# ezrakhuzadi/FFmpeg-hybrid

Hardware: AMD Instinct MI355X
Metric: decoded frames/sec (bit-exact) 4K VP9 Profile-0 @ 1/2/4/8 MI355X; % HBM roofline (higher is better)
Workload: dtype u8; 1 GPU; C3: 3840x2160 VP9 Profile-0 8-bit, 4 tile columns, all keyframes, 120 frames per GPU per step, pass-1 packets resident in HBM; global_batch=120, frames_per_gpu=120, parallelism=frame-sharded x1 (independent keyframes, no collective), streams_per_gpu=1, batches_in_flight=3

## Files before the change

### ffmpeg-hybrid_amd/__init__.py

```python
import collections
import ctypes
import os
import sys

import numpy as np

_HERE = os.path.dirname(os.path.abspath(__file__))
LIB_PATH = os.path.join(_HERE, "libvp9hip.so")

EINVAL = -22
ENOMEM = -12
ENOSYS = -38
EAGAIN = -11
EOF = -541478725
EINVALIDDATA = -1094995529
EEXTERNAL = -542398533
EBUG = -558323010

BS_64x64, BS_64x32, BS_32x64, BS_32x32, BS_32x16, BS_16x32, BS_16x16, BS_16x8, BS_8x16, \
    BS_8x8, BS_8x4, BS_4x8, BS_4x4 = range(13)


class Vp9HipUnavailable(RuntimeError):
    pass
# ... 180 lines not shown
                                     ctypes.POINTER(FramePacket)]
    L.vp9h_enc_defaults.argtypes = [ctypes.POINTER(EncParams)]
    L.vp9h_enc_defaults.restype = None
    L.vp9h_superframe_split.argtypes = [ctypes.c_void_p, ctypes.c_size_t, ctypes.POINTER(ctypes.c_size_t),
                                        ctypes.POINTER(ctypes.c_size_t), ctypes.c_int]
    L.vp9h_frame_type.argtypes = [ctypes.c_void_p, ctypes.c_size_t]
    L.vp9h_frame_peek.argtypes = [ctypes.c_void_p, ctypes.c_size_t, ctypes.POINTER(FrameInfo)]
    L.vp9hip_slot_stream_wait.argtypes = [vp, ctypes.c_int, ctypes.c_void_p]
    L.vp9h_ivf_probe.argtypes = [ctypes.c_void_p, ctypes.c_size_t]
    L.vp9h_ivf_read_header.argtypes = [ctypes.c_void_p, ctypes.c_size_t, ctypes.POINTER(IvfHeader)]
    L.vp9h_ivf_read_frame.argtypes = [ctypes.c_void_p, ctypes.c_size_t, ctypes.POINTER(ctypes.c_size_t),
                                      ctypes.POINTER(ctypes.c_void_p), ctypes.POINTER(ctypes.c_uint32),
                                      ctypes.POINTER(ctypes.c_int64), ctypes.POINTER(ctypes.c_int)]
    L.vp9h_ivf_write_header.argtypes = [ctypes.c_void_p, ctypes.c_int, ctypes.c_int, ctypes.c_uint32, ctypes.c_uint32,
                                        ctypes.c_uint32]
    L.vp9h_ivf_write_frame_header.argtypes = [ctypes.c_void_p, ctypes.c_uint32, ctypes.c_int64]
    L.vp9h_ivf_write_frame_header.restype = None
    L.vp9h_webm_probe.argtypes = [ctypes.c_void_p, ctypes.c_size_t]
    L.vp9h_webm_read_header.argtypes = [ctypes.c_void_p, ctypes.c_size_t, ctypes.POINTER(WebmInfo),
                                        ctypes.POINTER(WebmCursor)]
    L.vp9h_webm_read_frame.argtypes = [ctypes.c_void_p, ctypes.c_size_t, ctypes.POINTER(WebmCursor),
                                       ctypes.POINTER(ctypes.c_void_p), ctypes.POINTER(ctypes.c_uint32),
                                       ctypes.POINTER(ctypes.c_int64), ctypes.POINTER(ctypes.c_int)]
    L.vp9hip_decoder_defaults.argtypes = [ctypes.POINTER(DecoderParams)]
    L.vp9hip_decoder_defaults.restype = None
    L.vp9hip_decoder_open.argtypes = [ctypes.POINTER(DecoderParams), ctypes.POINTER(vp)]
    L.vp9hip_decoder_close.argtypes = [vp]
    L.vp9hip_decoder_close.restype = None
    L.vp9hip_decoder_context.argtypes = [vp]
    L.vp9hip_decoder_context.restype = vp
    L.vp9hip_decoder_send_packet.argtypes = [vp, ctypes.c_void_p, ctypes.c_size_t, ctypes.c_int64]
    L.vp9hip_decoder_receive_frame.argtypes = [vp, ctypes.POINTER(DecodedFrameInfo)]
    L.vp9hip_decoder_release.argtypes = [vp, ctypes.c_int]
    L.vp9hip_decoder_flush.argtypes = [vp]
    L.vp9h_stream_set_color.argtypes = [ctypes.c_void_p, ctypes.c_int, ctypes.c_int]
    L.vp9hip_out_layout.argtypes = [ctypes.POINTER(OutDesc), ctypes.c_int, ctypes.c_int, ctypes.c_int,
                                    ctypes.POINTER(ctypes.c_int64), ctypes.POINTER(ctypes.c_int64)]
    L.vp9hip_out_layout.restype = ctypes.c_int64
    L.vp9hip_out_coefs.argtypes = [ctypes.c_int] * 4 + [ctypes.POINTER(ctypes.c_int32), ctypes.POINTER(ctypes.c_int32)]
    L.vp9hip_convert_frames.argtypes = [vp, ctypes.POINTER(ctypes.c_int), ctypes.c_int, ctypes.POINTER(OutDesc),
                                        ctypes.c_void_p, ctypes.c_void_p]
    L.vp9hip_decoder_convert.argtypes = [vp, ctypes.POINTER(DecodedFrameInfo), ctypes.c_int, ctypes.c_int,
                                         ctypes.c_void_p, ctypes.c_int64, ctypes.c_int64, ctypes.c_void_p]
    L.vp9hip_convert_frames_scaled.argtypes = [vp, ctypes.POINTER(ctypes.c_int), ctypes.c_int, ctypes.POINTER(OutDesc),
                                               ctypes.c_int, ctypes.c_int, ctypes.c_void_p, ctypes.c_void_p]
    L.vp9hip_decoder_convert_scaled.argtypes = [vp, ctypes.POINTER(DecodedFrameInfo), ctypes.c_int, ctypes.c_int,
                                                ctypes.c_int, ctypes.c_int, ctypes.c_void_p, ctypes.c_int64,
                                                ctypes.c_int64, ctypes.c_void_p]
    L.vp9hip_resid4_host.argtypes = [ctypes.c_int] * 4 + [ctypes.c_void_p] * 3
    L.vp9hip_residn_host.argtypes = [ctypes.c_int] * 4 + [ctypes.c_void_p] * 3
    L.vp9hip_intra_job_host.argtypes = [ctypes.c_int] * 15 + [ctypes.POINTER(ctypes.c_int32)]
    L.vp9hip_intra_job_dev.argtypes = [ctypes.c_int] * 13 + [ctypes.POINTER(ctypes.c_int32)]
    L.vp9hip_plan_sched_host.argtypes = [ctypes.c_int] * 3 + [ctypes.c_void_p] * 4
    L.vp9hip_test_plan_records.argtypes = [vp, ctypes.c_int, ctypes.POINTER(ctypes.c_int)] + [ctypes.c_void_p] * 4
    _lib_handle = L
    return L


class IvfHeader(ctypes.Structure):
    _fields_ = [("fourcc", ctypes.c_char * 5), ("width", ctypes.c_int32), ("height", ctypes.c_int32),
                ("time_base_den", ctypes.c_uint32), ("time_base_num", ctypes.c_uint32),
                ("nb_frames", ctypes.c_uint32), ("header_size", ctypes.c_uint32)]


class WebmInfo(ctypes.Structure):
    _fields_ = [("doctype", ctypes.c_char * 16), ("codec_id", ctypes.c_char * 32), ("track", ctypes.c_uint64),
                ("width", ctypes.c_int32), ("height", ctypes.c_int32), ("timecode_scale", ctypes.c_uint64)]


class WebmCursor(ctypes.Structure):
    _fields_ = [("pos", ctypes.c_uint64), ("seg_end", ctypes.c_uint64), ("cluster_end", ctypes.c_uint64),
                ("track", ctypes.c_uint64), ("cluster_tc", ctypes.c_int64), ("block_pts", ctypes.c_int64),
                ("block_duration", ctypes.c_int64), ("cluster_unknown", ctypes.c_int32), ("keyframe", ctypes.c_int32),
                ("nlaces", ctypes.c_int32), ("lace_idx", ctypes.c_int32), ("lace_pos", ctypes.c_uint64),
                ("lace_size", ctypes.c_uint32 * 256)]


class DecoderParams(ctypes.Structure):
    _fields_ = [("device", ctypes.c_int32), ("max_batch", ctypes.c_int32), ("extra_bufs", ctypes.c_int32),
                ("max_width", ctypes.c_int32), ("max_height", ctypes.c_int32), ("parse_threads", ctypes.c_int32)]


class DecodedFrameInfo(ctypes.Structure):
    _fields_ = [("buf", ctypes.c_int32), ("width", ctypes.c_int32), ("height", ctypes.c_int32),
                ("bpp", ctypes.c_int32), ("ss_h", ctypes.c_int32), ("ss_v", ctypes.c_int32),
                ("pts", ctypes.c_int64), ("colorspace", ctypes.c_int32), ("full_range", ctypes.c_int32)]


class OutDesc(ctypes.Structure):
    _fields_ = [("format", ctypes.c_int32), ("colorspace", ctypes.c_int32), ("full_range", ctypes.c_int32),
                ("width", ctypes.c_int32), ("height", ctypes.c_int32), ("pitch", ctypes.c_int64),
                ("frame_stride", ctypes.c_int64)]


OUT_FORMATS = {"semiplanar": 0, "rgb24": 1, "rgbp_u8": 2, "rgbp_f16": 3}


def _check(fn, r):
    if r < 0:
        raise Vp9HipError(fn, r)
    return r


def resid4_host(bpp, tcode, txtp, eobs, coefs):
    hb = int(bpp > 8)
    coefs = np.ascontiguousarray(coefs, np.int32 if hb else np.int16)
    eobs = np.ascontiguousarray(eobs, np.uint8)
    n = len(eobs)
    assert coefs.shape == (n, 16)
    res = np.empty((n, 16), np.int32)
    _check("vp9hip_resid4_host", lib().vp9hip_resid4_host(hb, tcode, txtp, n, eobs.ctypes.data, coefs.ctypes.data,
                                                          res.ctypes.data))
    return res


def residn_host(bpp, tcode, txtp, eobs, coefs):
    hb = int(bpp > 8)
    coefs = np.ascontiguousarray(coefs, np.int32 if hb else np.int16)
    eobs = np.ascontiguousarray(eobs, np.uint16)
    n = len(eobs)
    nn = (4 << tcode) ** 2 if 1 <= tcode <= 3 else coefs.shape[1]
    assert coefs.shape == (n, nn)
    res = np.empty((n, nn), np.int32)
    _check("vp9hip_residn_host", lib().vp9hip_residn_host(hb, tcode, txtp, n, eobs.ctypes.data, coefs.ctypes.data,
                                                          res.ctypes.data))
    return res


def plan_sched_host(ss_h, ss_v, ja):
    ja = np.ascontiguousarray(ja, np.uint32)
    n = len(ja)
    order, passes, masks = np.empty(n, np.uint16), np.empty(max(n, 1), np.uint32), np.empty(n, np.uint32)
    npass = _check("vp9hip_plan_sched_host", lib().vp9hip_plan_sched_host(ss_h, ss_v, n, ja.ctypes.data, order.ctypes.data,
                                                                         passes.ctypes.data, masks.ctypes.data))
    return order, passes[:npass].copy(), masks


def intra_txfm_type(mode):
    return _check("vp9hip_intra_txfm_type", lib().vp9hip_intra_txfm_type(int(mode)))


IntraJob = collections.namedtuple("IntraJob", "slot have_top have_left ct cl trreal nd trx")


def intra_job_host(p, txs, mode, bx, by, x, y, pw4, tile_x0, cols, rows, ss_h, ss_v, ux0, uy0):
    out = (ctypes.c_int32 * 8)()
    _check("vp9hip_intra_job_host", lib().vp9hip_intra_job_host(p, txs, mode, bx, by, x, y, pw4, tile_x0, cols, rows,
                                                                ss_h, ss_v, ux0, uy0, out))
    return IntraJob(*out)


def intra_job_dev(p, txs, mode, sbx, sby, ux0, uy0, right, tile_sb0, cols, rows, ss_h, ss_v):
    out = (ctypes.c_int32 * 8)()
    _check("vp9hip_intra_job_dev", lib().vp9hip_intra_job_dev(p, txs, mode, sbx, sby, ux0, uy0, int(right), tile_sb0, cols,
                                                              rows, ss_h, ss_v, out))
    return IntraJob(*out)


def synth_params(width, height, bpp=8, **kw):
    p = SynthParams()
    lib().vp9hip_synth_defaults(ctypes.byref(p), width, height, bpp)
    for k, v in kw.items():
        if not hasattr(p, k):
            raise KeyError(k)
        if k == "seg" and isinstance(v, dict):
            v = seg_params(**v)
        setattr(p, k, v)
    return p


class SynthFrame:

    def __init__(self, params):
        self.params = params
        self.pkt = FramePacket()
        _check("vp9hip_synth_frame", lib().vp9hip_synth_frame(ctypes.byref(self.pkt), ctypes.byref(params)))

    def __del__(self):
        if getattr(self, "pkt", None) is not None and _lib_handle is not None:
            _lib_handle.vp9hip_synth_free(ctypes.byref(self.pkt))
            self.pkt = None

    @property
    def nbytes_coefs(self):
        return self.pkt.ncoefs * (2 if self.pkt.bpp == 8 else 4)

    def blocks(self):
        return [self.pkt.blocks[i] for i in range(self.pkt.nblocks)]
# ... 710 lines not shown
```

### ffmpeg-hybrid_amd/csrc/vp9hip_plan.hip

```cpp
#include <hip/hip_runtime.h>
#include <hipcub/hipcub.hpp>
#include <stdint.h>

#include "vp9hip_plan.h"

#define DEV __device__ __forceinline__

namespace {

enum { OP_ADD, OP_OR, OP_MAX };
template <int OP> DEV uint32_t dpp_op(uint32_t a, uint32_t b) { return OP == OP_OR ? (a | b) : OP == OP_MAX ? (a > b ? a : b) : (a + b); }
template <int OP> DEV uint32_t wscan_dpp(uint32_t v)
{
    v = dpp_op<OP>(v, (uint32_t) __builtin_amdgcn_update_dpp(0, (int) v, 0x111, 0xf, 0xf, true));
    v = dpp_op<OP>(v, (uint32_t) __builtin_amdgcn_update_dpp(0, (int) v, 0x112, 0xf, 0xf, true));
    v = dpp_op<OP>(v, (uint32_t) __builtin_amdgcn_update_dpp(0, (int) v, 0x114, 0xf, 0xf, true));
    v = dpp_op<OP>(v, (uint32_t) __builtin_amdgcn_update_dpp(0, (int) v, 0x118, 0xf, 0xf, true));
    v = dpp_op<OP>(v, (uint32_t) __builtin_amdgcn_update_dpp(0, (int) v, 0x142, 0xa, 0xf, false));
    v = dpp_op<OP>(v, (uint32_t) __builtin_amdgcn_update_dpp(0, (int) v, 0x143, 0xc, 0xf, false));
    return v;
}
DEV uint32_t wscan_incl(uint32_t v, int) { return wscan_dpp<OP_ADD>(v); }
DEV uint32_t rdl(uint32_t v, int l) { return (uint32_t) __builtin_amdgcn_readlane((int) v, l); }
DEV int rdl(int v, int l) { return __builtin_amdgcn_readlane(v, l); }
// ... 302 lines not shown
    ncoef = wsum(ncoef);
    wsync();
    uint32_t ib = 0;
    if (lane < 24)
#pragma unroll
        for (int j = 0; j < IBC; j++) ib |= ibw[lane * IBC + j];
    if (lane < 20) {
        const uint32_t ci = cnt_idx(D, F, G.seg, G.slot, lane >> 2, lane & 3);
        if (inb(D, ci, D.cap_cnt, 2u)) D.cnt[ci] = kcnt;
    }
    if (lane == 20) {
        const uint32_t ci = D.seg_pre1[G.seg] + D.slot_pos[G.slot];
        if (inb(D, ci, D.cap_cntm, 2u)) D.cntm[ci] = nmc;
    }
    if (lane < 24 && rec_ok) D.ibits[(size_t) G.slot * 24 + lane] = ib;
    if (lane == 0 && rec_ok) D.sb_tn[G.slot] = (uint32_t) T | (uint32_t) pl_min((int) (R.tot >> 20), JCAP) << 16;
    if (lane == 0 && inb(D, G.dord, D.nslots, 8u)) D.sb_ncoef[G.dord] = ncoef;
    if (st) plan_fail(D, F, st);
    PPT(2);
}

template <int JCAP> struct alignas(16) PlanLds {
    uint32_t ja[JCAP];
    union {
        uint16_t jmap[3][256];
        struct {
            union {
                uint32_t hgt[JCAP];
                uint16_t ord[JCAP];
            } h;
            uint16_t doff[JCAP + 1];
            union {
                uint16_t dep[4 * JCAP];
                struct {
                    uint32_t mk[JCAP];
                    uint32_t drow[64], dcol[64];
                } rd;
            } d;
            uint32_t hs[64];
            uint16_t tk[16];
        } b;
    } u;
};
static_assert(sizeof(uint16_t[3][256]) <= sizeof(uint32_t[256 + 2 * 64]), "the unit map fits the heights' region");
#define JM_ENT PL_JM_ENT

DEV uint32_t needs_of(uint32_t a)
{
    return (uint32_t) pl_slot_needs((int) ((a >> 8) & 15));
}
DEV uint32_t wor(uint32_t v) { return rdl(wscan_dpp<OP_OR>(v), 63); }

template <int SSH, int SSV>
DEV int pjob_sb(const PlanDev &D, const PlanFrame &F, uint32_t *ja)
{
    constexpr int CW = 16 >> SSH, CH = 16 >> SSV, JCAP = 256 + 2 * CW * CH, NCH = 6;
    const int s = blockIdx.x, lane = threadIdx.x;
    unsigned long long pt0 = D.prof ? clock64() : 0;
    const SbGeo G = sb_geo(F, s);
    const uint32_t slot = G.slot;
    uint32_t st = 0, bf = 0;
    if (slot >= D.nslots) bf |= 4u;
    if (G.dord >= D.nslots) bf |= 32u;
    const TxRec *rec = D.txrec + (size_t) slot * JCAP;
    TxRec x[NCH];
#pragma unroll
    for (int c = 0; c < NCH; c++) x[c].w = x[c].m = 0;
    if (!bf) x[0] = rec[lane];
    const uint32_t tn = bf ? 0u : D.sb_tn[slot];
    const uint32_t coef_sb = bf ? 0u : D.sb_coef0[G.dord];
    uint32_t rb = 0;
    if (lane < 20) {
        const uint32_t ci = cnt_idx(D, F, G.seg, slot, lane >> 2, lane & 3);
        if (ci < D.cap_cnt) rb = D.cnt0[ci];
        else bf |= 16u;
    }
    const int T = pl_min((int) (tn & 0xffff), JCAP), NJ = pl_min((int) (tn >> 16), JCAP);
    if (lane >= T) x[0].w = x[0].m = 0;
    const uint32_t rbase = slot * D.rcap;
    const uint16_t *nz16 = (const uint16_t *) D.nz;
    const int cols = F.mc.cols, rows = F.mc.rows, tx0l = G.tile_sb0 * 64;
    uint32_t carry = 0;
    unsigned long long ibytes = 0;
    int nj = 0;
    for (int g0 = 0; g0 < T; g0 += 64 * NCH) {
#pragma unroll
    for (int c = 0; c < NCH; c++)
        if (g0 || c) {
            x[c].w = x[c].m = 0;
            if (g0 + c * 64 + lane < T) x[c] = rec[g0 + c * 64 + lane];
        }
    PPT(3);
    uint32_t coef[NCH], nzv[NCH];
#pragma unroll
    for (int c = 0; c < NCH; c++) {
        if (g0 + c * 64 >= T) break;
        const uint32_t w = x[c].w, m = x[c].m;
        const uint32_t e0 = TXR_EOB(m), key = TXR_KEY(m);
        const uint32_t incl = wscan_incl(e0, lane);
        uint32_t cf = coef_sb + carry + incl - e0, e = e0;
        carry += rdl(incl, 63);
        if (TXR_EMIT(m) && cf + e > D.total_coefs) { st |= PLS_COEF; e = 0; cf = 0; x[c].m = m & ~2047u; }
        coef[c] = cf;
        nzv[c] = TXR_EMIT(m) ? nz16[key * 1025 + e] : 0u;
        const uint64_t mj = __ballot((w & TXR_JOB) != 0);
        if (w & TXR_JOB) {
            const int p = w & 3, txs = (w >> 2) & 3, ux0 = (w >> 12) & 15, uy0 = (w >> 16) & 15;
            const PlIntra pi = pl_intra_job_sb(p, txs, (int) ((w >> 8) & 15), (int) e0, G.sbx, G.sby, ux0, uy0,
                                               (w & TXR_RIGHT) != 0, tx0l, cols, rows, SSH, SSV);
            ja[nj + (int) mbcnt(mj)] = pi.a | (pi.trx ? JA_TRX : 0u);
        }
        nj += __popcll(mj);
    }
    PPT(4);
#pragma unroll
    for (int c = 0; c < NCH; c++) {
        if (g0 + c * 64 >= T) break;
        const uint32_t w = x[c].w, m = x[c].m, key = TXR_KEY(m);
        const uint32_t base = (uint32_t) __shfl((int) rb, (int) key);
        if (TXR_EMIT(m)) {
            const int p = w & 3, txs = (w >> 2) & 3, ux0 = (w >> 12) & 15, uy0 = (w >> 16) & 15;
            const int sh = p ? SSH : 0, sv = p ? SSV : 0;
            const bool intra = (w & TXR_JOB) != 0;
            uint32_t dst;
            if (intra) dst = rbase + pl_resid_unit(p, ux0, uy0, SSH, SSV);
            else {
                dst = (uint32_t) ((size_t) (G.sby * (64 >> sv) + uy0 * 4) * F.pitch[p ? 1 : 0] + G.sbx * (64 >> sh) + ux0 * 4);
                ibytes += (unsigned long long) (2 * (16 << (2 * txs)) * F.bypp);
            }
            const uint32_t ptx = (uint32_t) p | (key >> 2) << 2 | (intra ? 0u : 1u) << 5 | (key & 3) << 6;
            const uint32_t pos = base + TXR_RANK(m);
            if (pos < D.cap_rjobs)
                *(uint4 *) &D.rjobs[pos] = make_uint4(coef[c], dst, TXR_EOB(m) | (uint32_t) (F.frame & 0xffff) << 16,
                                                      ptx | nzv[c] << 8);
            else bf |= 64u;
        }
    }
    PPT(5);
    }
    for (int d = 32; d; d >>= 1) ibytes += __shfl_xor(ibytes, d);
    if (lane == 0 && ibytes) {
        if ((uint32_t) F.frame < D.nframes) atomicAdd(&D.fbytes[2 * F.frame], ibytes);
        else bf |= 2048u;
    }
    bf = wor(bf);
    if (lane == 0 && bf) { atomicOr(&D.status[1], bf); atomicOr(&D.status[0], PLS_BOUNDS); }
    st = wor(st);
    if (lane == 0 && st) plan_fail(D, F, st);
    return pl_min(nj, NJ);
}
static_assert(sizeof(RJob) == 16 && offsetof(RJob, eob) == 8 && offsetof(RJob, frame) == 10 && offsetof(RJob, ptx) == 12 &&
              offsetof(RJob, nzc) == 13 && offsetof(RJob, nzr) == 14, "pjob_sb stores an RJob as one uint4");

template <int SSH, int SSV>
DEV void plan_sb(const PlanDev &D, const PlanFrame &F, PlanLds<256 + 2 * (16 >> SSH) * (16 >> SSV)> &S, int nj)
{
    constexpr int CW = 16 >> SSH, CH = 16 >> SSV, JCAP = 256 + 2 * CW * CH, NCH = JCAP / 64;
    const int s = blockIdx.x, lane = threadIdx.x;
    unsigned long long pt0 = D.prof ? clock64() : 0;
    const SbGeo G = sb_geo(F, s);
    const uint32_t slot = G.slot;
    const uint32_t rbase = slot * D.rcap;
    uint32_t st = 0;
    const int NJ = pl_min(nj, JCAP);
    for (int i = lane; i < 3 * 256 / 8; i += 64) ((uint4 *) &S.u.jmap[0][0])[i] = make_uint4(~0u, ~0u, ~0u, ~0u);
    wsync();
    PPT(6);
    for (int j = lane; j < NJ; j += 64) {
        const uint32_t a = S.ja[j];
        const int p = a & 3, step = 1 << ((a >> 2) & 3), ux0 = (a >> 12) & 15, uy0 = (a >> 16) & 15;
        const int units = p ? CW : 16, unitsv = p ? CH : 16;
        if (ux0 + step <= units) {
            uint16_t *row = &S.u.jmap[p][uy0 * 16 + ux0];
            for (int v = 0; v < step && uy0 + v < unitsv; v++, row += 16) {
                const uint32_t b = JM_ENT(j, 0, step - 1 - v);
                auto e2 = [&](uint32_t r) { return (b | r << 10) | (b | (r - 1) << 10) << 16; };
                if (step == 1) *row = (uint16_t) b;
                else if (step == 2) *(uint32_t *) row = e2(1);
                else if (step == 4) *(uint2 *) row = make_uint2(e2(3), e2(1));
                else *(uint4 *) row = make_uint4(e2(7), e2(5), e2(3), e2(1));
            }
        } else {
            for (int v = uy0; v < uy0 + step && v < unitsv; v++)
                for (int u = ux0; u < ux0 + step && u < units; u++)
                    S.u.jmap[p][v * 16 + u] = (uint16_t) JM_ENT(j, ux0 + step - 1 - u, uy0 + step - 1 - v);
        }
    }
    wsync();
    PPT(7);

    auto deps_of = [&](int j, auto fn) {
        const uint32_t a = S.ja[j];
        const int p = a & 3, ts = (a >> 2) & 3, ux0 = (a >> 12) & 15, uy0 = (a >> 16) & 15;
        return pl_deps(S.u.jmap[p], j, ux0, uy0, 1 << ts, (int) needs_of(a), (a & JA_TRX) ? 1 : 0, p ? CW : 16, p ? CH : 16, fn);
    };
    uint32_t mreg[NCH];
#pragma unroll
    for (int c = 0; c < NCH; c++) mreg[c] = 0;
    {
        uint32_t carry = 0;
        for (int c = 0; c < NJ; c += 64) {
            const int j = c + lane;
            const uint32_t cap = j < NJ ? 2u * (1u << ((S.ja[j] >> 2) & 3)) + 2u : 0u;
            const uint32_t incl = wscan_incl(cap, lane);
            const uint32_t off = carry + incl - cap;
            uint32_t mk = 0;
            if (j < NJ) {
                uint32_t k = off;
                if (off + cap <= 4u * JCAP) mk = deps_of(j, [&](int d) { if (k < off + cap) S.u.b.d.dep[k++] = (uint16_t) d; });
                else st |= PLS_SCHED;
                S.u.b.doff[j] = (uint16_t) (off >> 1 | (k - off) << 11);
            }
#pragma unroll
            for (int cc = 0; cc < NCH; cc++)
                if (c == cc * 64) mreg[cc] = mk;
            carry += rdl(incl, 63);
        }
        wsync();
        for (int j = lane; j < NJ; j += 64) S.u.b.h.hgt[j] = 1;
    }
    wsync();
    PPT(8);
    for (int c = ((NJ - 1) & ~63); c >= 0; c -= 64) {
        const int j = c + lane;
        const uint32_t dw = j < NJ ? S.u.b.doff[j] : 0u;
        const int k0 = (int) (dw & 2047) << 1, k1 = k0 + (int) (dw >> 11);
        for (int it = 0; it < 65; it++) {
            bool ch = false;
            if (j < NJ) {
                const uint32_t h1 = S.u.b.h.hgt[j] + 1;
                for (int k = k0; k < k1; k++) {
                    const int d = S.u.b.d.dep[k];
                    if (S.u.b.h.hgt[d] < h1) { atomicMax(&S.u.b.h.hgt[d], h1); ch |= d >= c; }
                }
            }
            wsync();
            if (!__any(ch)) break;
        }
    }
    PPT(9);
    int hreg[NCH];
#pragma unroll
    for (int c = 0; c < NCH; c++) {
        const int j = c * 64 + lane;
        hreg[c] = j < NJ ? pl_min((int) S.u.b.h.hgt[j], 63) : -1;
        if (j < NJ) S.u.b.d.rd.mk[j] = mreg[c];
    }
    S.u.b.d.rd.drow[lane] = S.u.b.d.rd.dcol[lane] = 0;
    S.u.b.hs[lane] = 0;
    wsync();
#pragma unroll
    for (int c = 0; c < NCH; c++)
        if (hreg[c] >= 0) atomicAdd(&S.u.b.hs[hreg[c]], 1u);
    wsync();
    {
        const uint32_t v = S.u.b.hs[63 - lane];
        const uint32_t incl = wscan_incl(v, lane);
        wsync();
        S.u.b.hs[63 - lane] = incl - v;
        wsync();
#pragma unroll
        for (int c = 0; c < NCH; c++) {
            if (c * 64 >= NJ) break;
            const int j = c * 64 + lane;
            const int h = hreg[c];
            uint64_t m = __ballot(h >= 0);
#pragma unroll
            for (int b = 0; b < 6; b++) {
                const uint64_t bal = __ballot((h >> b) & 1);
                m &= ((h >> b) & 1) ? bal : ~bal;
            }
            const uint32_t rank = __builtin_amdgcn_mbcnt_hi((uint32_t) (m >> 32), __builtin_amdgcn_mbcnt_lo((uint32_t) m, 0u));
            uint32_t base = 0;
            if (h >= 0 && rank == 0) base = atomicAdd(&S.u.b.hs[h], (uint32_t) __popcll(m));
            base = (uint32_t) __shfl((int) base, __ffsll((unsigned long long) m) - 1);
            if (h >= 0) S.u.b.h.ord[base + rank] = (uint16_t) j;
        }
    }
    wsync();
    PPT(10);
    uint32_t *gpass = D.passes + (size_t) slot * JCAP;
    PJob *gjob = D.pjobs + (size_t) slot * JCAP;
    int done = 0, npass = 0;
    uint32_t jwreg[NCH], mkreg[NCH];
    uint32_t pend = 0;
#pragma unroll
    for (int c = 0; c < NCH; c++) {
        const int pos = c * 64 + lane;
        jwreg[c] = mkreg[c] = 0;
        if (pos < NJ) {
            const uint32_t j = S.u.b.h.ord[pos], a = S.ja[j];
// ... 60 lines not shown
        sr.frame = (uint32_t) F.frame; sr.sbx = (uint16_t) G.sbx; sr.sby = (uint16_t) G.sby;
        sr.tile_x0 = (uint16_t) (G.tile_sb0 << 3);
        sr.flags = F.intra ? 0 : 1;
        D.sbs[slot] = sr;
        WGRec w;
        w.job0 = slot * JCAP; w.pass0 = slot * JCAP;
        w.njobs = (uint16_t) done; w.npass = (uint16_t) npass;
        w.sb[0] = slot;
        D.wgs[slot] = w;
    }
    PPT(11);

    uint32_t dmask = 0;
    if (F.levels && !F.intra)
        for (int j = lane; j < NJ; j += 64) {
            const uint32_t a = S.ja[j];
            const int p = a & 3, ts = (a >> 2) & 3, ux0 = (a >> 12) & 15, uy0 = (a >> 16) & 15;
            const int units = p ? CW : 16, unitsv = p ? CH : 16;
            const int fx = G.sbx * units + ux0, fy = G.sby * unitsv + uy0;
            pl_cross_reads(ux0, uy0, fx, fy, 1 << ts, (int) needs_of(a), (a & JA_TRX) ? 1 : 0, [&](int ux, int uy) {
                if (ux < 0 || uy < 0 || ux >= F.sb_cols * units) return;
                const int nx = ux / units, ny = uy / unitsv, u = ux - nx * units, v = uy - ny * unitsv;
                const uint32_t ns = F.slot0 + (uint32_t) (ny * F.sb_cols + nx);
                if (!((D.ibits[(size_t) ns * 24 + p * 8 + (v >> 1)] >> ((v & 1) * 16 + u)) & 1)) return;
                dmask |= nx < G.sbx ? (ny < G.sby ? 8u : 2u) : 4u;
            });
        }
    dmask = wor(dmask);
    PPT(12);


    if (lane == 0) {
        const uint32_t has = done > 0;
        D.sb_info[slot] = has | dmask;
        if (D.static_lists) {
            if (!has && G.mine) st |= PLS_SCHED;
            D.sb_kpos[slot] = (uint32_t) npass;
        } else if (has && !(F.levels && !F.intra)) {
            const uint32_t key = F.key0 + (uint32_t) ((G.sbx - G.tile_sb0) + G.sby);
            D.sb_key[slot] = key;
            D.sb_kpos[slot] = inb(D, key, D.nkeys, 1024u) ? atomicAdd(&D.key_cnt[key], 1u) : 0u;
        }
    }
    st = wor(st);
    if (lane == 0 && st) plan_fail(D, F, st);
    PPT(13);
}
template <int SSH, int SSV>
__global__ __launch_bounds__(64) void k_pjplan(PlanDev D)
{
    __shared__ PlanLds<256 + 2 * (16 >> SSH) * (16 >> SSV)> S;
    const PlanFrame F = D.frames[blockIdx.y];
    if ((int) blockIdx.x >= F.sb_cols * F.sb_rows) return;
    const int nj = pjob_sb<SSH, SSV>(D, F, S.ja);
    wsync();
    plan_sb<SSH, SSV>(D, F, S, nj);
}

template <int SSH, int SSV>
__global__ __launch_bounds__(64) void k_plmc(PlanDev D)
{
    const PlanFrame &F = D.frames[blockIdx.y];
    const int s = blockIdx.x, lane = threadIdx.x;
    if (F.intra || s >= F.sb_cols * F.sb_rows) return;
    const SbGeo G = sb_geo(F, s);
    uint32_t st = 0, b0;
    const int nb = sb_blocks(D, G.slot, b0, st);
    const uint32_t ci = D.seg_pre1[G.seg] + D.slot_pos[G.slot];
    const uint32_t base = inb(D, ci, D.cap_cntm, 16u) ? D.cntm0[ci] : 0u;
    vp9h_block b;
    bool mc = false;
    if (lane < nb) {
        b = load_block(&D.blocks[b0 + lane]);
        mc = G.mine && !b.intra && mc_refs_ok(b, F.mc);
    }
    const uint32_t n = mc ? (uint32_t) pl_mc_block(b, F.mc, 0, [](const McUnit &) {}) : 0u;
    const uint32_t incl = wscan_incl(n, lane);
    uint32_t o = base + incl - n;
    unsigned long long mbytes = 0;
    if (mc)
        pl_mc_block(b, F.mc, (uint32_t) F.frame, [&](const McUnit &m) {
            if (inb(D, o, D.cap_mcs, 512u)) D.mcs[o] = m;
            o++;
            mbytes += (unsigned long long) m.w * m.h * F.bypp * (1 + m.nref);
        });
    for (int d = 32; d; d >>= 1) mbytes += __shfl_xor(mbytes, d);
    if (lane == 0 && mbytes && inb(D, (uint32_t) F.frame, D.nframes, 2048u)) atomicAdd(&D.fbytes[2 * F.frame + 1], mbytes);
}

template <int SSH, int SSV>
__global__ __launch_bounds__(64) void k_pllf(PlanDev D)
{
    __shared__ uint32_t lfm[2][2][8];
    __shared__ uint8_t lfl[64];
    __shared__ uint32_t prog[LF_PROG_BYTES / 4];
    const PlanFrame &F = D.frames[blockIdx.y];
    const int s = blockIdx.x, lane = threadIdx.x;
    if (!F.filter_level || s >= F.sb_cols * F.sb_rows) return;
    const SbGeo G = sb_geo(F, s);
    const int cols = F.mc.cols, rows = F.mc.rows;
    uint32_t st = 0, b0;
    const int nb = sb_blocks(D, G.slot, b0, st);
    if (lane < 32) (&lfm[0][0][0])[lane] = 0;
    lfl[lane] = 0;
    for (int i = lane; i < LF_PROG_BYTES / 4; i += 64) prog[i] = 0;
    wsync();
    if (lane < nb) {
        const vp9h_block b = load_block(&D.blocks[b0 + lane]);
        if (const int lvl = pl_lf_level(b, F.lflvl, F.filter_level)) {
// ... 229 lines not shown
```

### ffmpeg-hybrid_amd/csrc/vp9hip_planlogic.h

```cpp
#ifndef VP9HIP_PLANLOGIC_H
#define VP9HIP_PLANLOGIC_H
#include <stdint.h>
#include "../../include/vp9hip.h"
#include "vp9hip_work.h"

#define PL_HD __host__ __device__ static inline

PL_HD int pl_bwh(int i, int bs, int d)
{
    const uint64_t lw = 0x494936e4ull, lh = 0x20a29a71cull;
    const int l = (int) (((d ? lh : lw) >> (3 * bs)) & 7) - i;
    return 1 << (l > 0 ? l : 0);
}

PL_HD int pl_field(uint64_t packed, int i, int bits) { return (int) ((packed >> (bits * i)) & ((1u << bits) - 1)); }

PL_HD int pl_min(int a, int b) { return a < b ? a : b; }
PL_HD int pl_max(int a, int b) { return a > b ? a : b; }
PL_HD int pl_clamp(int v, int lo, int hi) { return v < lo ? lo : v > hi ? hi : v; }
PL_HD int pl_rdiv(int a, int b) { return (a >= 0 ? a + (b >> 1) : a - (b >> 1)) / b; }

PL_HD int pl_tile_of(int sbx, int sb_cols, int log2, int *tile_sb0)
{
    int t = 0, s0 = 0;
// ... 85 lines not shown
template <class F>
PL_HD void pl_local_reads(int ux0, int uy0, int n4, int nd, int trx, int units, int unitsv, F fn)
{
    if (uy0 > 0) {
        const int u0 = (nd & 4) ? ux0 - 1 : ux0, u1 = (nd & 2) ? ux0 + n4 + trx : ux0;
        for (int u = u0; u < u1; u++)
            if (u >= 0 && u < units) fn((uy0 - 1) * 16 + u);
    }
    if (ux0 > 0 && (nd & 1))
        for (int v = uy0; v < uy0 + n4; v++)
            if (v < unitsv) fn(v * 16 + ux0 - 1);
}

PL_HD int pl_slot_needs(int slot) { return pl_field(0x21371a777a12ull, slot, 4); }

#define PL_JM_ENT(j, r, b) ((uint32_t) (j) | (uint32_t) (r) << 10 | (uint32_t) (b) << 13)
#define PL_JM_NONE 0xffffu

template <class F>
PL_HD uint32_t pl_deps(const uint16_t *jm, int j, int ux0, int uy0, int n4, int nd, int trx, int units, int unitsv, F fn)
{
    uint32_t mk = 0;
    int tl = -1;
    if (uy0 > 0) {
        const int u1 = pl_min((nd & 2) ? ux0 + n4 + trx : ux0, units);
        int u = (nd & 4) ? ux0 - 1 : ux0;
        if (u < 0) u = 0;
        const uint16_t *row = jm + (uy0 - 1) * 16;
        while (u < u1) {
            const uint32_t e = row[u];
            if (e == PL_JM_NONE) { u++; continue; }
            const int d = (int) (e & 1023), r = pl_min((int) ((e >> 10) & 7), u1 - 1 - u);
            if (u == ux0 - 1) tl = d;
            if (d < j) { fn(d); mk |= ((2u << r) - 1u) << u; }
            u += (int) ((e >> 10) & 7) + 1;
        }
    }
    if (ux0 > 0 && (nd & 1)) {
        const int v1 = pl_min(uy0 + n4, unitsv);
        int v = uy0;
        const uint16_t *col = jm + ux0 - 1;
        while (v < v1) {
            const uint32_t e = col[v * 16];
            if (e == PL_JM_NONE) { v++; continue; }
            const int d = (int) (e & 1023), b = pl_min((int) (e >> 13), v1 - 1 - v);
            if (d < j) {
                if (d != tl) fn(d);
                mk |= ((2u << b) - 1u) << (16 + v);
            }
            v += (int) (e >> 13) + 1;
        }
    }
    return mk;
}

template <class F>
PL_HD void pl_cross_reads(int ux0, int uy0, int fx, int fy, int n4, int nd, int trx, F fn)
{
    if (uy0 == 0 && (nd & 6)) {
        const int u0 = (nd & 4) ? -1 : 0, u1 = (nd & 2) ? n4 + trx : 0;
        for (int u = u0; u < u1; u++) fn(fx + u, fy - 1);
    } else if (ux0 == 0 && (nd & 4)) {
        fn(fx - 1, fy - 1);
    }
    if (ux0 == 0 && (nd & 1))
        for (int v = 0; v < n4; v++) fn(fx - 1, fy + v);
}

template <class OR>
PL_HD void pl_lf_mask_edges(OR or_, int ss_h, int ss_v, int row7, int col7, int w, int h, int col_end, int row_end,
                            int tx, int skip_inter)
{
    const unsigned wide_col[2] = { 0x11, 0x01 }, wide_row[2] = { 0x03, 0x07 };
    if (tx == 0 && (ss_v | ss_h)) {
        if (h == ss_v) { if (row7 & 1) return; if (!row_end) h += 1; }
        if (w == ss_h) { if (col7 & 1) return; if (!col_end) w += 1; }
    }
    const unsigned t = 1u << col7, m_col = (t << w) - t;
    if (tx == 0 && !skip_inter) {
        const unsigned m8 = m_col & wide_col[ss_h], m4 = m_col - m8;
        for (int y = row7; y < h + row7; y++) {
            const int id = 2 - !(y & wide_row[ss_v]);
            or_(0, y, 1, m8);
            or_(0, y, 2, m4);
            or_(1, y, id, ((ss_h & ss_v) && (col_end & 1) && (y & 1)) ? (t << (w - 1)) - t : m_col);
            if (!ss_h) or_(0, y, 3, m_col);
            if (!ss_v) or_(1, y, 3, (ss_h && (col_end & 1)) ? (t << (w - 1)) - t : m_col);
        }
        return;
    }
    if (!skip_inter) {
        const uint32_t masks = 0x011155ffu;
        const int id = tx == 1;
        int l2 = tx + ss_h - 1;
        const unsigned m_row = m_col & ((masks >> (8 * l2)) & 255u);
        if (ss_h && tx > 1 && (w ^ (w - 1)) == 1) {
            const unsigned m16 = ((t << (w - 1)) - t) & ((masks >> (8 * l2)) & 255u), m8 = m_row - m16;
            for (int y = row7; y < h + row7; y++) { or_(0, y, 0, m16); or_(0, y, 1, m8); }
        } else {
            for (int y = row7; y < h + row7; y++) or_(0, y, id, m_row);
        }
        l2 = tx + ss_v - 1;
        const int step = 1 << l2;
        int y;
        if (ss_v && tx > 1 && (h ^ (h - 1)) == 1) {
            for (y = row7; y < h + row7 - 1; y += step) or_(1, y, 0, m_col);
// ... 274 lines not shown
```

### ffmpeg-hybrid_amd/csrc/vp9hip_runtime.cpp

```cpp
#include <hip/hip_runtime.h>

#include <algorithm>
#include <atomic>
#include <chrono>
#include <condition_variable>
#include <functional>
#include <memory>
#include <mutex>
#include <thread>
#include <array>
#include <cstdio>
#include <cstdlib>
#include <cstring>
#include <string>
#include <vector>

#pragma clang diagnostic ignored "-Wunused-result"
#pragma clang diagnostic ignored "-Wunused-value"

#include "../../include/vp9hip.h"
#include "vp9_tables.h"
#include "vp9hip_work.h"
#include "vp9hip_planlogic.h"
#include "vp9hip_plan.h"
// ... 2817 lines not shown
                jm[(size_t) (q.p * 256 + v * 16 + u)] = (uint16_t) PL_JM_ENT(j, q.ux0 + q.n4 - 1 - u, q.uy0 + q.n4 - 1 - v);
    }
    std::vector<std::vector<int>> prod((size_t) nj);
    for (int j = 0; j < nj; j++) {
        const J &q = job[(size_t) j];
        const uint32_t a = ja[j];
        const uint32_t mk = pl_deps(&jm[(size_t) q.p * 256], j, q.ux0, q.uy0, q.n4, pl_slot_needs((int) ((a >> 8) & 15)),
                                    (int) ((a >> 30) & 1), q.p ? CW : 16, q.p ? CH : 16, [](int) {});
        if (masks) masks[j] = mk;
        for (int b = 0; b < 32; b++) {
            if (!((mk >> b) & 1)) continue;
            const int unit = b < 16 ? (q.uy0 - 1) * 16 + b : (b - 16) * 16 + q.ux0 - 1;
            const int d = jm[(size_t) (q.p * 256 + unit)] & 1023;
            if (d >= j) return -2;
            if (std::find(prod[(size_t) j].begin(), prod[(size_t) j].end(), d) == prod[(size_t) j].end()) prod[(size_t) j].push_back(d);
        }
    }
    std::vector<int> h((size_t) nj, 1), pos((size_t) nj), pass_of((size_t) nj, -1);
    for (int j = nj - 1; j >= 0; j--)
        for (int d : prod[(size_t) j]) h[(size_t) d] = std::max(h[(size_t) d], h[(size_t) j] + 1);
    for (int j = 0; j < nj; j++) pos[(size_t) j] = j;
    std::stable_sort(pos.begin(), pos.end(), [&](int x, int y) { return std::min(h[(size_t) x], 63) > std::min(h[(size_t) y], 63); });
    int done = 0, npass = 0;
    while (done < nj) {
        int budget = 64;
        std::vector<int> tk;
        for (int c = 0; c < nj && budget >= 4; c += 64) {
            int sum = 0;
            for (int i = c; i < std::min(c + 64, nj); i++) {
                const int j = pos[(size_t) i];
                if (pass_of[(size_t) j] >= 0) continue;
                bool ready = true;
                for (int d : prod[(size_t) j]) ready = ready && pass_of[(size_t) d] >= 0 && pass_of[(size_t) d] < npass;
                if (!ready) continue;
                if (sum + 4 * job[(size_t) j].n4 > budget) break;
                sum += 4 * job[(size_t) j].n4;
                tk.push_back(j);
            }
            budget -= sum;
        }
        if (tk.empty()) return -2;
        for (int j : tk) pass_of[(size_t) j] = npass;
        uint32_t cnt[4] = { 0, 0, 0, 0 };
        int at = done;
        for (int n4 = 8; n4; n4 >>= 1)
            for (int j : tk)
                if (job[(size_t) j].n4 == n4) { order[at++] = (uint16_t) j; cnt[n4 == 8 ? 3 : n4 == 4 ? 2 : n4 == 2 ? 1 : 0]++; }
        passes[npass++] = (uint32_t) done << 14 | cnt[0] << 9 | cnt[1] << 5 | cnt[2] << 2 | cnt[3];
        done = at;
    }
    return npass;
}

extern "C" int vp9hip_test_plan_records(vp9hip_ctx *c, int cap_slots, int *jcap, uint32_t *sbs, uint32_t *wgs,
                                        uint32_t *passes, uint32_t *jobs_a)
{
    if (!c) return VP9HIP_EINVAL;
    Staged &s = c->stg;
    if (!s.dev || !s.planned || !s.arena || !s.nslots || s.jcap <= 0) return VP9HIP_EINVAL;
    static_assert(sizeof(SBRec) == 12 && sizeof(WGRec) == 16 && sizeof(PJob) == 8, "the layouts vp9hip.h describes");
    const size_t ns = s.nslots, jc = (size_t) s.jcap;
    if (jcap) *jcap = s.jcap;
    if (!sbs && !wgs && !passes && !jobs_a) return (int) ns;
    if (cap_slots < 0 || (size_t) cap_slots < ns) return VP9HIP_EINVAL;
    hipSetDevice(c->dev);
    HIPCHK(hipDeviceSynchronize());
    if (sbs) HIPCHK(hipMemcpy(sbs, s.arena + s.o_sbs, ns * sizeof(SBRec), hipMemcpyDeviceToHost));
    if (wgs) HIPCHK(hipMemcpy(wgs, s.arena + s.o_wgs, ns * sizeof(WGRec), hipMemcpyDeviceToHost));
    if (passes) HIPCHK(hipMemcpy(passes, s.arena + s.o_passes, ns * jc * 4, hipMemcpyDeviceToHost));
    if (jobs_a) {
        std::vector<PJob> pj(ns * jc);
        HIPCHK(hipMemcpy(pj.data(), s.arena + s.o_pjobs, ns * jc * sizeof(PJob), hipMemcpyDeviceToHost));
        for (size_t k = 0; k < ns * jc; k++) jobs_a[k] = pj[k].a;
    }
    return (int) ns;
}

extern "C" int vp9hip_device_info(int device, char *pci_bus_id, int len, char *name, int name_len)
{
    int n = 0;
    if (hipGetDeviceCount(&n) != hipSuccess || device < 0 || device >= n) return VP9HIP_ENOSYS;
    if (pci_bus_id && len > 0) HIPCHK(hipDeviceGetPCIBusId(pci_bus_id, len, device));
    if (name && name_len > 0) {
        hipDeviceProp_t p;
        HIPCHK(hipGetDeviceProperties(&p, device));
        snprintf(name, (size_t) name_len, "%s (%s)", p.name, p.gcnArchName);
    }
    return 0;
}

extern "C" int vp9hip_set_batch_slot(vp9hip_ctx *c, int slot)
{
    if (!c || slot < 0 || slot >= MAX_SLOTS) return VP9HIP_EINVAL;
    if (slot != c->slot) {
        if (c->slot_streams) {
            hipSetDevice(c->dev);
            if (!slot_streams_make(c, slot)) return VP9HIP_EEXTERNAL;
        }
        std::swap(c->stg, c->sl[c->slot]);
        std::swap(c->stg, c->sl[slot]);
        if (c->slot_streams) {
            c->st = c->sst[slot];
            for (int i = 0; i < MAX_GROUPS - 1; i++) c->xst[i] = c->sxst[slot][i];
        }
        c->slot = slot;
    }
// ... 158 lines not shown
```

### include/vp9hip.h

```cpp
#ifndef VP9HIP_H
#define VP9HIP_H

#include <stddef.h>
#include <stdint.h>

#ifdef __cplusplus
extern "C" {
#endif

#define VP9HIP_ABI_VERSION 5

#define VP9HIP_EINVAL       (-22)
#define VP9HIP_ENOMEM       (-12)
#define VP9HIP_ENOSYS       (-38)
#define VP9HIP_EINVALIDDATA (-1094995529)
#define VP9HIP_EEXTERNAL    (-542398533)
#define VP9HIP_EBUG         (-558323010)
#define VP9HIP_EAGAIN       (-11)
#define VP9HIP_EOF          (-541478725)

enum { VP9H_BS_64x64, VP9H_BS_64x32, VP9H_BS_32x64, VP9H_BS_32x32, VP9H_BS_32x16,
       VP9H_BS_16x32, VP9H_BS_16x16, VP9H_BS_16x8, VP9H_BS_8x16, VP9H_BS_8x8,
       VP9H_BS_8x4, VP9H_BS_4x8, VP9H_BS_4x4, VP9H_N_BS };
enum { VP9H_TX_4X4, VP9H_TX_8X8, VP9H_TX_16X16, VP9H_TX_32X32 };
enum { VP9H_FILTER_SMOOTH, VP9H_FILTER_REGULAR, VP9H_FILTER_SHARP, VP9H_FILTER_BILINEAR };
enum { VP9H_NEARESTMV = 10, VP9H_NEARMV = 11, VP9H_ZEROMV = 12, VP9H_NEWMV = 13 };

typedef struct vp9h_block {
    uint16_t row, col;
    uint8_t  bs;
    uint8_t  tx, uvtx;
    uint8_t  skip;
    uint8_t  intra, comp;
    uint8_t  seg_id;
    uint8_t  filter;
    uint8_t  mode[4];
    uint8_t  uvmode;
    uint8_t  ref[2];
    uint8_t  pad0;
    int16_t  mv[4][2][2];
} vp9h_block;

typedef struct vp9h_frame {
    int32_t  width, height;
    uint8_t  bpp;
    uint8_t  ss_h, ss_v;
    uint8_t  keyframe, intraonly;
    uint8_t  lossless;
    uint8_t  filter_level;
    uint8_t  sharpness;
    uint8_t  log2_tile_cols;
    uint8_t  log2_tile_rows;
    uint8_t  pad0[2];
    uint8_t  lflvl[8][4][2];
    int32_t  ref_w[3], ref_h[3];
    uint32_t nblocks;
    uint32_t neobs;
    uint64_t ncoefs;
    const vp9h_block *blocks;
    const uint16_t   *eobs;
    const void       *coefs;
} vp9h_frame;

typedef struct vp9hip_ctx vp9hip_ctx;

int  vp9hip_open(int device, vp9hip_ctx **out);
void vp9hip_close(vp9hip_ctx *ctx);
void vp9hip_test_hooks(int reject_batch, uint32_t lfr_spin);
int  vp9hip_test_plan_records(vp9hip_ctx *ctx, int cap_slots, int *jcap, uint32_t *sbs, uint32_t *wgs,
                              uint32_t *passes, uint32_t *jobs_a);
int  vp9hip_plan_sched_host(int ss_h, int ss_v, int nj, const uint32_t *ja, uint16_t *order, uint32_t *passes,
                            uint32_t *masks);

int  vp9hip_configure(vp9hip_ctx *ctx, int width, int height, int bpp, int ss_h, int ss_v,
                      int nbufs);

int  vp9hip_submit_frame(vp9hip_ctx *ctx, const vp9h_frame *pkt, int out_buf,
                         const int ref_buf[3]);

int  vp9hip_stage_batch(vp9hip_ctx *ctx, const vp9h_frame *pkts, int n, const int *out_bufs);
int  vp9hip_run_batch(vp9hip_ctx *ctx);
int  vp9hip_stage_batch_refs(vp9hip_ctx *ctx, const vp9h_frame *pkts, int n, const int *out_bufs,
                             const int *ref_bufs);

#define VP9HIP_PART_RECON 0
#define VP9HIP_PART_LF    1
int  vp9hip_stage_batch_tiles(vp9hip_ctx *ctx, const vp9h_frame *pkts, int n, const int *out_bufs,
                              const int *ref_bufs, int tile_lo, int tile_hi);
int  vp9hip_batch_phases(vp9hip_ctx *ctx);
int  vp9hip_batch_groups(vp9hip_ctx *ctx);
int  vp9hip_phase_frames(vp9hip_ctx *ctx, int phase, int *frames, int cap);
int  vp9hip_run_phase(vp9hip_ctx *ctx, int phase, int part);
int64_t vp9hip_stripe(vp9hip_ctx *ctx, int frame, int tile_lo, int tile_hi, void *dev, int to_frame);

#define VP9HIP_MAX_SLOTS 4
#define VP9HIP_PIPELINE_SLOTS 3
int  vp9hip_set_batch_slot(vp9hip_ctx *ctx, int slot);
int  vp9hip_sync_slot(vp9hip_ctx *ctx, int slot);
int  vp9hip_batch_frame_status(vp9hip_ctx *ctx, int slot, int *status, int cap);
int  vp9hip_slot_stream_wait(vp9hip_ctx *ctx, int slot, void *stream);
int  vp9hip_slot_busy(vp9hip_ctx *ctx, int slot);
int  vp9hip_sync(vp9hip_ctx *ctx);

int  vp9hip_download_frame(vp9hip_ctx *ctx, int buf, uint8_t *const planes[3],
                           const ptrdiff_t linesize[3]);
int  vp9hip_frame_device(vp9hip_ctx *ctx, int buf, void *planes[3], ptrdiff_t linesize[3],
                         int *width, int *height, void **stream);

enum { VP9HIP_OUT_SEMIPLANAR,
       VP9HIP_OUT_RGB24,
       VP9HIP_OUT_RGBP_U8,
       VP9HIP_OUT_RGBP_F16 };
typedef struct vp9hip_out_desc {
    int32_t format;
    int32_t colorspace;
    int32_t full_range;
    int32_t width, height;
    int64_t pitch;
    int64_t frame_stride;
} vp9hip_out_desc;
int64_t vp9hip_out_layout(const vp9hip_out_desc *d, int bpp, int ss_h, int ss_v,
                          int64_t *pitch, int64_t plane_offset[3]);
int     vp9hip_out_coefs(int colorspace, int full_range, int bpp, int out_bits, int32_t c[5], int32_t *shift);
int  vp9hip_convert_frames(vp9hip_ctx *ctx, const int *bufs, int n, const vp9hip_out_desc *d,
                           void *dst_dev, void *stream);
// ... 193 lines not shown
```

Before: 13140 frames/s.

## Cache first four dependency indices in registers for height propagation loop

The longest-path height propagation in the per-superblock planner now preloads each job's first four dependency indices into packed registers once per chunk, then runs branch-free atomicMax updates on them each iteration. Only jobs with more than four deps fall back to the LDS walk. Empty dependency slots point at a spare LDS slot so the atomics need no guards. The shared logic moves into a header template with a host reference implementation for testing, and superblock geometry is computed once and passed to both phases. Trade-offs: unconditional atomics on padding slots and extra register pressure.

```diff
diff --git a/ffmpeg-hybrid_amd/__init__.py b/ffmpeg-hybrid_amd/__init__.py
--- a/ffmpeg-hybrid_amd/__init__.py
+++ b/ffmpeg-hybrid_amd/__init__.py
@@ -256,6 +256,7 @@
     L.vp9hip_intra_job_host.argtypes = [ctypes.c_int] * 15 + [ctypes.POINTER(ctypes.c_int32)]
     L.vp9hip_intra_job_dev.argtypes = [ctypes.c_int] * 13 + [ctypes.POINTER(ctypes.c_int32)]
     L.vp9hip_plan_sched_host.argtypes = [ctypes.c_int] * 3 + [ctypes.c_void_p] * 4
+    L.vp9hip_plan_heights_host.argtypes = [ctypes.c_int] * 3 + [ctypes.c_void_p] * 2
     L.vp9hip_test_plan_records.argtypes = [vp, ctypes.c_int, ctypes.POINTER(ctypes.c_int)] + [ctypes.c_void_p] * 4
     _lib_handle = L
     return L
@@ -338,6 +339,13 @@
     npass = _check("vp9hip_plan_sched_host", lib().vp9hip_plan_sched_host(ss_h, ss_v, n, ja.ctypes.data, order.ctypes.data,
                                                                          passes.ctypes.data, masks.ctypes.data))
     return order, passes[:npass].copy(), masks
+
+
+def plan_heights_host(ss_h, ss_v, ja):
+    ja = np.ascontiguousarray(ja, np.uint32)
+    heights = np.empty(len(ja), np.uint32)
+    _check("vp9hip_plan_heights_host", lib().vp9hip_plan_heights_host(ss_h, ss_v, len(ja), ja.ctypes.data, heights.ctypes.data))
+    return heights
 
 
 def intra_txfm_type(mode):
diff --git a/ffmpeg-hybrid_amd/csrc/vp9hip_plan.hip b/ffmpeg-hybrid_amd/csrc/vp9hip_plan.hip
--- a/ffmpeg-hybrid_amd/csrc/vp9hip_plan.hip
+++ b/ffmpeg-hybrid_amd/csrc/vp9hip_plan.hip
@@ -378,12 +378,11 @@
 DEV uint32_t wor(uint32_t v) { return rdl(wscan_dpp<OP_OR>(v), 63); }
 
 template <int SSH, int SSV>
-DEV int pjob_sb(const PlanDev &D, const PlanFrame &F, uint32_t *ja)
+DEV int pjob_sb(const PlanDev &D, const PlanFrame &F, const SbGeo &G, uint32_t *ja)
 {
     constexpr int CW = 16 >> SSH, CH = 16 >> SSV, JCAP = 256 + 2 * CW * CH, NCH = 6;
-    const int s = blockIdx.x, lane = threadIdx.x;
+    const int lane = threadIdx.x;
     unsigned long long pt0 = D.prof ? clock64() : 0;
-    const SbGeo G = sb_geo(F, s);
     const uint32_t slot = G.slot;
     uint32_t st = 0, bf = 0;
     if (slot >= D.nslots) bf |= 4u;
@@ -479,12 +478,11 @@
               offsetof(RJob, nzc) == 13 && offsetof(RJob, nzr) == 14, "pjob_sb stores an RJob as one uint4");
 
 template <int SSH, int SSV>
-DEV void plan_sb(const PlanDev &D, const PlanFrame &F, PlanLds<256 + 2 * (16 >> SSH) * (16 >> SSV)> &S, int nj)
+DEV void plan_sb(const PlanDev &D, const PlanFrame &F, const SbGeo &G, PlanLds<256 + 2 * (16 >> SSH) * (16 >> SSV)> &S, int nj)
 {
     constexpr int CW = 16 >> SSH, CH = 16 >> SSV, JCAP = 256 + 2 * CW * CH, NCH = JCAP / 64;
-    const int s = blockIdx.x, lane = threadIdx.x;
+    const int lane = threadIdx.x;
     unsigned long long pt0 = D.prof ? clock64() : 0;
-    const SbGeo G = sb_geo(F, s);
     const uint32_t slot = G.slot;
     const uint32_t rbase = slot * D.rcap;
     uint32_t st = 0;
@@ -535,7 +533,7 @@
                 uint32_t k = off;
                 if (off + cap <= 4u * JCAP) mk = deps_of(j, [&](int d) { if (k < off + cap) S.u.b.d.dep[k++] = (uint16_t) d; });
                 else st |= PLS_SCHED;
-                S.u.b.doff[j] = (uint16_t) (off >> 1 | (k - off) << 11);
+                S.u.b.doff[j] = (uint16_t) (k > off ? off >> 1 | (k - off) << 11 : 0u);
             }
 #pragma unroll
             for (int cc = 0; cc < NCH; cc++)
@@ -547,22 +545,13 @@
     }
     wsync();
     PPT(8);
-    for (int c = ((NJ - 1) & ~63); c >= 0; c -= 64) {
-        const int j = c + lane;
-        const uint32_t dw = j < NJ ? S.u.b.doff[j] : 0u;
-        const int k0 = (int) (dw & 2047) << 1, k1 = k0 + (int) (dw >> 11);
-        for (int it = 0; it < 65; it++) {
-            bool ch = false;
-            if (j < NJ) {
-                const uint32_t h1 = S.u.b.h.hgt[j] + 1;
-                for (int k = k0; k < k1; k++) {
-                    const int d = S.u.b.d.dep[k];
-                    if (S.u.b.h.hgt[d] < h1) { atomicMax(&S.u.b.h.hgt[d], h1); ch |= d >= c; }
-                }
-            }
-            wsync();
-            if (!__any(ch)) break;
-        }
+    {
+        uint32_t *hgt = S.u.b.h.hgt;
+        const uint32_t spare = (uint32_t) (S.u.b.hs - hgt);
+        auto each = [&](auto fn) { const bool r = fn(lane, 0); wsync(); return __any(r) != 0; };
+        auto amax = [&](uint32_t i, uint32_t v) { return atomicMax(&hgt[i], v); };
+        for (int c = (D.dbg & 16) ? -1 : ((NJ - 1) & ~63); c >= 0; c -= 64)
+            pl_heights_chunk<1>(hgt, S.u.b.d.dep, S.u.b.doff, c, NJ, spare, each, amax);
     }
     PPT(9);
     int hreg[NCH];
@@ -729,9 +718,10 @@
     __shared__ PlanLds<256 + 2 * (16 >> SSH) * (16 >> SSV)> S;
     const PlanFrame F = D.frames[blockIdx.y];
     if ((int) blockIdx.x >= F.sb_cols * F.sb_rows) return;
-    const int nj = pjob_sb<SSH, SSV>(D, F, S.ja);
-    wsync();
-    plan_sb<SSH, SSV>(D, F, S, nj);
+    const SbGeo G = sb_geo(F, blockIdx.x);
+    const int nj = pjob_sb<SSH, SSV>(D, F, G, S.ja);
+    wsync();
+    plan_sb<SSH, SSV>(D, F, G, S, nj);
 }
 
 template <int SSH, int SSV>
diff --git a/ffmpeg-hybrid_amd/csrc/vp9hip_planlogic.h b/ffmpeg-hybrid_amd/csrc/vp9hip_planlogic.h
--- a/ffmpeg-hybrid_amd/csrc/vp9hip_planlogic.h
+++ b/ffmpeg-hybrid_amd/csrc/vp9hip_planlogic.h
@@ -161,6 +161,45 @@
         }
     }
     return mk;
+}
+
+template <int NL, class EACH, class AMAX>
+PL_HD void pl_heights_chunk(uint32_t *hgt, const uint16_t *dep, const uint16_t *doff, int c, int nj, uint32_t spare, EACH each,
+                            AMAX amax)
+{
+    uint32_t e01[NL], e23[NL];
+    const bool longl = each([&](int lane, int r) {
+        const int j = c + lane;
+        const uint32_t dw = j < nj ? doff[j] : 0u, sp = spare + (uint32_t) lane;
+        const int k0 = (int) (dw & 2047) << 1, n = (int) (dw >> 11);
+        const uint32_t d0 = dep[k0], d1 = dep[k0 + 1], d2 = dep[k0 + 2], d3 = dep[k0 + 3];
+        e01[r] = (n > 0 ? d0 : sp) | (n > 1 ? d1 : sp) << 16;
+        e23[r] = (n > 2 ? d2 : sp) | (n > 3 ? d3 : sp) << 16;
+        return n > 4;
+    });
+    for (int it = 0; it < 65; it++) {
+        const bool rose = each([&](int lane, int r) {
+            const uint32_t j = (uint32_t) (c + lane), lo = (uint32_t) c;
+            const uint32_t h1 = hgt[(int) j < nj ? j : spare + (uint32_t) lane] + 1;
+            const uint32_t d0 = e01[r] & 0xffff, d1 = e01[r] >> 16, d2 = e23[r] & 0xffff, d3 = e23[r] >> 16;
+            const uint32_t o0 = amax(d0, h1), o1 = amax(d1, h1), o2 = amax(d2, h1), o3 = amax(d3, h1);
+            const uint32_t jl = j - lo;
+            const uint32_t x0 = d0 - lo < jl ? o0 : ~0u, x1 = d1 - lo < jl ? o1 : ~0u;
+            const uint32_t x2 = d2 - lo < jl ? o2 : ~0u, x3 = d3 - lo < jl ? o3 : ~0u;
+            const uint32_t xa = x0 < x1 ? x0 : x1, xb = x2 < x3 ? x2 : x3;
+            bool ch = (xa < xb ? xa : xb) < h1;
+            if (longl && (int) j < nj) {
+                const uint32_t dw = doff[j];
+                const int k0 = (int) (dw & 2047) << 1, k1 = k0 + (int) (dw >> 11);
+                for (int k = k0 + 4; k < k1; k++) {
+                    const uint32_t d = dep[k];
+                    if (hgt[d] < h1) { amax(d, h1); ch |= d >= lo; }
+                }
+            }
+            return ch;
+        });
+        if (!rose) break;
+    }
 }
 
 template <class F>
diff --git a/ffmpeg-hybrid_amd/csrc/vp9hip_runtime.cpp b/ffmpeg-hybrid_amd/csrc/vp9hip_runtime.cpp
--- a/ffmpeg-hybrid_amd/csrc/vp9hip_runtime.cpp
+++ b/ffmpeg-hybrid_amd/csrc/vp9hip_runtime.cpp
@@ -2893,6 +2893,40 @@
     return npass;
 }
 
+extern "C" int vp9hip_plan_heights_host(int ss_h, int ss_v, int nj, const uint32_t *ja, uint32_t *heights)
+{
+    if ((ss_h | ss_v | 1) != 1 || nj < 0 || nj > pl_rcap(ss_h, ss_v) || (nj && (!ja || !heights))) return -1;
+    const int CW = 16 >> ss_h, CH = 16 >> ss_v, JCAP = pl_rcap(ss_h, ss_v);
+    std::vector<uint16_t> jm(3 * 256, (uint16_t) PL_JM_NONE), dep((size_t) 4 * JCAP, 0), doff((size_t) JCAP + 1, 0);
+    for (int j = 0; j < nj; j++) {
+        const uint32_t a = ja[j];
+        const int p = a & 3, n4 = 1 << ((a >> 2) & 3), ux0 = (a >> 12) & 15, uy0 = (a >> 16) & 15;
+        if (p > 2 || (ux0 & (n4 - 1)) || (uy0 & (n4 - 1)) || ux0 >= (p ? CW : 16) || uy0 >= (p ? CH : 16)) return -1;
+        for (int v = uy0; v < uy0 + n4 && v < (p ? CH : 16); v++)
+            for (int u = ux0; u < ux0 + n4 && u < (p ? CW : 16); u++)
+                jm[(size_t) (p * 256 + v * 16 + u)] = (uint16_t) PL_JM_ENT(j, ux0 + n4 - 1 - u, uy0 + n4 - 1 - v);
+    }
+    uint32_t off = 0;
+    for (int j = 0; j < nj; j++) {
+        const uint32_t a = ja[j], cap = 2u * (1u << ((a >> 2) & 3)) + 2u;
+        const int p = a & 3;
+        if (off + cap > 4u * (uint32_t) JCAP) return -2;
+        uint32_t k = off;
+        pl_deps(&jm[(size_t) p * 256], j, (a >> 12) & 15, (a >> 16) & 15, 1 << ((a >> 2) & 3), pl_slot_needs((int) ((a >> 8) & 15)),
+                (int) ((a >> 30) & 1), p ? CW : 16, p ? CH : 16, [&](int d) { if (k < off + cap) dep[k++] = (uint16_t) d; });
+        doff[(size_t) j] = (uint16_t) (k > off ? off >> 1 | (k - off) << 11 : 0u);
+        off += cap;
+    }
+    std::vector<uint32_t> hgt((size_t) JCAP + 128, 0);
+    for (int j = 0; j < nj; j++) hgt[(size_t) j] = 1;
+    auto each = [&](auto fn) { bool any = false; for (int l = 0; l < 64; l++) any |= fn(l, l); return any; };
+    auto amax = [&](uint32_t i, uint32_t v) { const uint32_t old = hgt[i]; hgt[i] = std::max(old, v); return old; };
+    for (int c = (nj - 1) & ~63; c >= 0; c -= 64)
+        pl_heights_chunk<64>(hgt.data(), dep.data(), doff.data(), c, nj, (uint32_t) JCAP + 64, each, amax);
+    for (int j = 0; j < nj; j++) heights[j] = hgt[(size_t) j];
+    return 0;
+}
+
 extern "C" int vp9hip_test_plan_records(vp9hip_ctx *c, int cap_slots, int *jcap, uint32_t *sbs, uint32_t *wgs,
                                         uint32_t *passes, uint32_t *jobs_a)
 {
diff --git a/include/vp9hip.h b/include/vp9hip.h
--- a/include/vp9hip.h
+++ b/include/vp9hip.h
@@ -71,6 +71,7 @@
                               uint32_t *passes, uint32_t *jobs_a);
 int  vp9hip_plan_sched_host(int ss_h, int ss_v, int nj, const uint32_t *ja, uint16_t *order, uint32_t *passes,
                             uint32_t *masks);
+int  vp9hip_plan_heights_host(int ss_h, int ss_v, int nj, const uint32_t *ja, uint32_t *heights);
 
 int  vp9hip_configure(vp9hip_ctx *ctx, int width, int height, int bpp, int ss_h, int ss_v,
                       int nbufs);
```

Result: faster. 13770 frames/s, median of 6 (+4.8%).
